# ivanacollg/MPC_CollisionAvoidance

Measured on AMD Instinct MI355X. Metric: batched SQP-RTI solves/sec (USV, N=40 horizon, 10 obstacles), higher is better.
Workload: dtype f64

## Files before the change

### include/usvmpc.h

```cpp
#ifndef USVMPC_H
#define USVMPC_H

#include <stddef.h>

#ifdef __cplusplus
extern "C" {
#endif

#define USVMPC_NX_MAX 14
#define USVMPC_NU_MAX 2
#define USVMPC_NY_MAX 16
#define USVMPC_K_MAX 32

enum { USVMPC_MODEL_USV = 0,
       USVMPC_MODEL_GUIDANCE_CA1 = 1,
       USVMPC_MODEL_PF_CA = 2,
       USVMPC_MODEL_GENERATED = 3 };

enum { USVMPC_HPIPM_BALANCE = 0, USVMPC_HPIPM_SPEED = 1, USVMPC_HPIPM_ROBUST = 2, USVMPC_HPIPM_R04 = 3 };

enum { USVMPC_E_ARG = -1, USVMPC_E_FIELD = -2, USVMPC_E_STAGE = -3, USVMPC_E_SIZE = -4,
       USVMPC_E_HIP = -5, USVMPC_E_NODEVICE = -6 };

typedef struct usvmpc_desc {
// ... 13 lines not shown
    double uh[USVMPC_K_MAX];
    int soft;
    double lsh[USVMPC_K_MAX], ush[USVMPC_K_MAX];
    double zl[USVMPC_K_MAX], zu[USVMPC_K_MAX], Zl[USVMPC_K_MAX], Zu[USVMPC_K_MAX];
    int qp_iter_max;
    double mu0, thr0, tol_stat, tol_eq, tol_ineq, tol_comp, alpha_min;
    int sbx[USVMPC_NX_MAX];
    double lsbx[USVMPC_NX_MAX], usbx[USVMPC_NX_MAX];
    double zl_bx[USVMPC_NX_MAX], zu_bx[USVMPC_NX_MAX], Zl_bx[USVMPC_NX_MAX], Zu_bx[USVMPC_NX_MAX];
    int sim_num_steps;
    int nlp_max_iter;
    double nlp_tol_stat, nlp_tol_eq, nlp_tol_ineq, nlp_tol_comp;
    int hpipm_mode;
    int cond_pred_corr;
    double cpc_factor;
} usvmpc_desc;

typedef struct usvmpc_handle usvmpc_handle;

int usvmpc_model_dims(int model, int *nx, int *nu);
void usvmpc_default_options(usvmpc_desc *d);
int usvmpc_hpipm_profile(usvmpc_desc *d, int mode);

int usvmpc_create(const usvmpc_desc *d, usvmpc_handle **out);
int usvmpc_destroy(usvmpc_handle *h);

int usvmpc_set(usvmpc_handle *h, const char *field, int stage, const double *v, size_t n);
int usvmpc_get(usvmpc_handle *h, const char *field, int stage, double *out, size_t n);
int usvmpc_obstacles_step(usvmpc_handle *h, double T);
int usvmpc_get_int(usvmpc_handle *h, const char *field, int *out);
// ... 3 lines not shown
int usvmpc_solve_async(usvmpc_handle *h);
int usvmpc_sync(usvmpc_handle *h);

int usvmpc_get_device_ptr(usvmpc_handle *h, const char *field, void **dptr);
int usvmpc_last_kernel_ms(usvmpc_handle *h, float *linearize_ms, float *qp_ms);
int usvmpc_kernel_ms(usvmpc_handle *h, int n, float *linearize_ms, float *qp_ms);
int usvmpc_tick_ms(usvmpc_handle *h, int n, float *ms);
int usvmpc_fail_counts(usvmpc_handle *h, int n, int *counts);
int usvmpc_unconverged_counts(usvmpc_handle *h, int n, int *counts);
int usvmpc_unconverged_total(usvmpc_handle *h, long long *total);
int usvmpc_handover_counts(usvmpc_handle *h, int n, int *counts);
int usvmpc_followup_ms(usvmpc_handle *h, int n, float *ms);
int usvmpc_handover_co_counts(usvmpc_handle *h, int n, int *finished, int *timeouts);
int usvmpc_pipeline_stats(usvmpc_handle *h, long *used, long *discarded);
int usvmpc_lin_pair_launches(usvmpc_handle *h, long *launches);
int usvmpc_last_mapping(usvmpc_handle *h, int *mapping);
int usvmpc_advance(usvmpc_handle *h, double sigma, unsigned long long seed);
int usvmpc_set_stream(usvmpc_handle *h, void *stream);
int usvmpc_set_option(usvmpc_handle *h, const char *name, double value);
int usvmpc_guidance_reset(usvmpc_handle *h, const double *waypoints, int npts, const double *psi);
int usvmpc_guidance_prepare(usvmpc_handle *h, const double *vel_uv, const double *pose, const double *obstacles,
                            const int *n_obstacles, int lmax);
int usvmpc_guidance_sense(usvmpc_handle *h, const double *pose, const double *world, int n_world, double max_radius,
                          double *obstacles, int *n_obstacles);
int usvmpc_guidance_publish(usvmpc_handle *h, double *heading, double *r_des, double *speed, double *ye, int *active);
int usvmpc_guidance_state(usvmpc_handle *h, int *wp_index, float *past_psied);
int usvmpc_pf_reset(usvmpc_handle *h, const double *waypoints, int npts);
int usvmpc_pf_world(usvmpc_handle *h, const double *world, int n_world, double max_radius);
int usvmpc_pf_prepare(usvmpc_handle *h, const double *vel_uvr, const double *pose);
int usvmpc_pf_publish(usvmpc_handle *h, double *thr_port, double *thr_stbd, double *Tx, double *Tz, float *e_u, float *e_ye, double *speed,
// ... 34 lines not shown
```

### mpc_collisionavoidance_amd/_capi.py

```python
import ctypes as C
import os
import sys

import numpy as np

NXM, NUM, NYM, KM = 14, 2, 16, 32
MODEL_IDS = {"usv_model": 0, "usv_model_guidance_ca1": 1, "usv_model_pf_ca": 2}
MODEL_DIMS = {0: (5, 2), 1: (8, 1), 2: (14, 2)}

_dp = C.POINTER(C.c_double)
_ip = C.POINTER(C.c_int)


class Desc(C.Structure):
    _fields_ = [("model", C.c_int), ("N", C.c_int), ("Tf", C.c_double), ("K", C.c_int),
                ("batch", C.c_int), ("device", C.c_int),
                ("W", C.c_double * (NYM * NYM)), ("W_e", C.c_double * (NXM * NXM)),
                ("Vx", C.c_double * (NYM * NXM)), ("Vu", C.c_double * (NYM * NUM)),
                ("Vx_e", C.c_double * (NXM * NXM)),
                ("nbu", C.c_int), ("idxbu", C.c_int * NUM), ("lbu", C.c_double * NUM), ("ubu", C.c_double * NUM),
                ("nbx", C.c_int), ("idxbx", C.c_int * NXM), ("lbx", C.c_double * NXM), ("ubx", C.c_double * NXM),
                ("uh", C.c_double * KM), ("soft", C.c_int),
                ("lsh", C.c_double * KM), ("ush", C.c_double * KM),
                ("zl", C.c_double * KM), ("zu", C.c_double * KM), ("Zl", C.c_double * KM), ("Zu", C.c_double * KM),
                ("qp_iter_max", C.c_int), ("mu0", C.c_double), ("thr0", C.c_double),
                ("tol_stat", C.c_double), ("tol_eq", C.c_double), ("tol_ineq", C.c_double),
                ("tol_comp", C.c_double), ("alpha_min", C.c_double),
                ("sbx", C.c_int * NXM), ("lsbx", C.c_double * NXM), ("usbx", C.c_double * NXM),
                ("zl_bx", C.c_double * NXM), ("zu_bx", C.c_double * NXM), ("Zl_bx", C.c_double * NXM), ("Zu_bx", C.c_double * NXM),
                ("sim_num_steps", C.c_int), ("nlp_max_iter", C.c_int),
                ("nlp_tol_stat", C.c_double), ("nlp_tol_eq", C.c_double), ("nlp_tol_ineq", C.c_double),
                ("nlp_tol_comp", C.c_double),
                ("hpipm_mode", C.c_int), ("cond_pred_corr", C.c_int), ("cpc_factor", C.c_double)]


class SimDesc(C.Structure):
    _fields_ = [("model", C.c_int), ("batch", C.c_int), ("device", C.c_int), ("T", C.c_double), ("num_steps", C.c_int),
                ("sens_forw", C.c_int)]


HPIPM_MODES = {"BALANCE": 0, "SPEED": 1, "ROBUST": 2, "R04": 3}


def lib_path():
    return os.environ.get("USVMPC_LIB") or os.path.join(os.path.dirname(os.path.abspath(__file__)), "csrc", "libusvmpc.so")


loaded_before_torch = False

EXPORTS = ["usvmpc_model_dims", "usvmpc_default_options", "usvmpc_hpipm_profile", "usvmpc_create", "usvmpc_destroy",
           "usvmpc_set", "usvmpc_get", "usvmpc_get_int", "usvmpc_solve", "usvmpc_solve_sqp", "usvmpc_solve_async",
           "usvmpc_sync", "usvmpc_get_device_ptr", "usvmpc_last_kernel_ms", "usvmpc_kernel_ms", "usvmpc_tick_ms", "usvmpc_fail_counts", "usvmpc_unconverged_counts", "usvmpc_unconverged_total", "usvmpc_handover_counts", "usvmpc_handover_co_counts", "usvmpc_followup_ms", "usvmpc_pipeline_stats", "usvmpc_lin_pair_launches", "usvmpc_last_mapping",
           "usvmpc_advance", "usvmpc_set_stream", "usvmpc_set_option", "usvmpc_calibrate_traffic", "usvmpc_guidance_reset", "usvmpc_guidance_prepare", "usvmpc_guidance_sense",
           "usvmpc_guidance_publish", "usvmpc_guidance_state", "usvmpc_device_bytes", "usvmpc_last_error",
           "usvmpc_debug_model_eval", "usvmpc_debug_obstacle_eval",
           "usvmpc_sim_create", "usvmpc_sim_destroy", "usvmpc_sim_set", "usvmpc_sim_solve", "usvmpc_sim_get", "usvmpc_sim_get_device_ptr",
           "usvmpc_sim_set_stream", "usvmpc_sim_last_error", "usvmpc_advance_sim", "usvmpc_obstacles_step",
           "usvmpc_pf_reset", "usvmpc_pf_world", "usvmpc_pf_prepare", "usvmpc_pf_publish", "usvmpc_pf_state",
           "usvmpc_pf_world_vel", "usvmpc_pf_world_step", "usvmpc_pf_world_read"]


_libs = {}


def load(path):
    global loaded_before_torch
    path = os.path.abspath(path)
# ... 21 lines not shown
    L.usvmpc_solve_sqp.argtypes = [C.c_void_p, _ip]
    L.usvmpc_solve_async.argtypes = [C.c_void_p]
    L.usvmpc_sync.argtypes = [C.c_void_p]
    L.usvmpc_get_device_ptr.argtypes = [C.c_void_p, C.c_char_p, C.POINTER(C.c_void_p)]
    L.usvmpc_last_kernel_ms.argtypes = [C.c_void_p, C.POINTER(C.c_float), C.POINTER(C.c_float)]
    L.usvmpc_kernel_ms.argtypes = [C.c_void_p, C.c_int, C.POINTER(C.c_float), C.POINTER(C.c_float)]
    L.usvmpc_tick_ms.argtypes = [C.c_void_p, C.c_int, C.POINTER(C.c_float)]
    L.usvmpc_fail_counts.argtypes = [C.c_void_p, C.c_int, _ip]
    L.usvmpc_unconverged_counts.argtypes = [C.c_void_p, C.c_int, _ip]
    L.usvmpc_handover_counts.argtypes = [C.c_void_p, C.c_int, _ip]
    L.usvmpc_unconverged_total.argtypes = [C.c_void_p, C.POINTER(C.c_longlong)]
    L.usvmpc_handover_co_counts.argtypes = [C.c_void_p, C.c_int, _ip, _ip]
    L.usvmpc_followup_ms.argtypes = [C.c_void_p, C.c_int, C.POINTER(C.c_float)]
    L.usvmpc_pipeline_stats.argtypes = [C.c_void_p, C.POINTER(C.c_long), C.POINTER(C.c_long)]
    L.usvmpc_lin_pair_launches.argtypes = [C.c_void_p, C.POINTER(C.c_long)]
    L.usvmpc_last_mapping.argtypes = [C.c_void_p, C.POINTER(C.c_int)]
    L.usvmpc_advance.argtypes = [C.c_void_p, C.c_double, C.c_ulonglong]
    L.usvmpc_set_stream.argtypes = [C.c_void_p, C.c_void_p]
    L.usvmpc_set_option.argtypes = [C.c_void_p, C.c_char_p, C.c_double]
    L.usvmpc_calibrate_traffic.argtypes = [C.c_void_p, C.c_int, _dp, _dp]
    L.usvmpc_guidance_reset.argtypes = [C.c_void_p, _dp, C.c_int, _dp]
    L.usvmpc_guidance_prepare.argtypes = [C.c_void_p, _dp, _dp, _dp, _ip, C.c_int]
    L.usvmpc_guidance_sense.argtypes = [C.c_void_p, _dp, _dp, C.c_int, C.c_double, _dp, _ip]
    L.usvmpc_guidance_publish.argtypes = [C.c_void_p, _dp, _dp, _dp, _dp, _ip]
    L.usvmpc_guidance_state.argtypes = [C.c_void_p, _ip, C.POINTER(C.c_float)]
    _fp = C.POINTER(C.c_float)
    L.usvmpc_pf_reset.argtypes = [C.c_void_p, _dp, C.c_int]
    L.usvmpc_pf_world.argtypes = [C.c_void_p, _dp, C.c_int, C.c_double]
    L.usvmpc_pf_prepare.argtypes = [C.c_void_p, _dp, _dp]
    L.usvmpc_pf_publish.argtypes = [C.c_void_p, _dp, _dp, _dp, _dp, _fp, _fp, _dp, _ip]
# ... 193 lines not shown
```

### mpc_collisionavoidance_amd/acados_template.py

```python
import ctypes as C

import numpy as np

from . import _capi


class SymVec:

    def __init__(self, n, names=None):
        self.n = int(n)
        self.names = list(names) if names is not None else ["v%d" % i for i in range(self.n)]

    def size(self):
        return (self.n, 1)

    @property
    def shape(self):
        return (self.n, 1)

    def __len__(self):
        return self.n

    def __sub__(self, other):
        return self
# ... 280 lines not shown
            return np.zeros(0)
        a = (C.c_float * (n - 1))()
        self._check(self._lib.usvmpc_tick_ms(self._h, n, a))
        return np.array(a[:])

    def fail_counts(self, n):
        a = (C.c_int * n)()
        self._check(self._lib.usvmpc_fail_counts(self._h, n, a))
        return np.array(a[:])

    def pipeline_stats(self):
        a, b = C.c_long(), C.c_long()
        self._check(self._lib.usvmpc_pipeline_stats(self._h, C.byref(a), C.byref(b)))
        return a.value, b.value

    def lin_pair_launches(self):
        a = C.c_long()
        self._check(self._lib.usvmpc_lin_pair_launches(self._h, C.byref(a)))
        return a.value

    def last_mapping(self):
        a = C.c_int()
        self._check(self._lib.usvmpc_last_mapping(self._h, C.byref(a)))
        return a.value

    def unconverged_counts(self, n):
        a = (C.c_int * n)()
        self._check(self._lib.usvmpc_unconverged_counts(self._h, n, a))
        return np.array(a[:])

# ... 357 lines not shown
```

### mpc_collisionavoidance_amd/csrc/gfx950/lanes.hpp

```cpp
#pragma once
#include <hip/hip_runtime.h>

#define USV_DEV __device__ __forceinline__

namespace lanes {

constexpr int GROUP = 16;

USV_DEV int lane() { return (int)(threadIdx.x & 15u); }
USV_DEV long group_linear() { return (long)blockIdx.x * (long)(blockDim.x >> 4) + (long)(threadIdx.x >> 4); }

template <int CTRL>
USV_DEV double dpp_mov(double v)
{
    const long l = __builtin_bit_cast(long, v);
    const long r = __builtin_amdgcn_update_dpp(0L, l, CTRL, 0xf, 0xf, true);
    return __builtin_bit_cast(double, r);
}

template <int K>
USV_DEV double bcast(double v)
{
    static_assert(K >= 0 && K < 16, "lane index");
    return dpp_mov<0x150 + K>(v);
// ... 191 lines not shown
    USV_DEV Planes(const double *base, unsigned nbytes, unsigned voff_) : voff(voff_)
    {
        rsrc = __builtin_amdgcn_make_buffer_rsrc(const_cast<double *>(base), 0, (int)nbytes, 0x00020000);
    }
    USV_DEV double ld(int plane) const
    {
        typedef unsigned u2 __attribute__((ext_vector_type(2)));
        const u2 v = __builtin_amdgcn_raw_buffer_load_b64(rsrc, (int)(voff + (unsigned)(plane * 128)), 0, PLANE_LOAD_AUX);
        return __builtin_bit_cast(double, v);
    }
    USV_DEV void st(int plane, double x) const
    {
        typedef unsigned u2 __attribute__((ext_vector_type(2)));
        __builtin_amdgcn_raw_buffer_store_b64(__builtin_bit_cast(u2, x), rsrc, (int)(voff + (unsigned)(plane * 128)), 0, PLANE_STORE_AUX);
    }
};

template <int NENT, int ROWS = 4, bool PERWAVE = false>
struct Xpose {
    USV_DEV static double *area()
    {
        __shared__ double s[NENT * ROWS];
        return s;
    }
    USV_DEV static unsigned row() { return PERWAVE ? (ROWS == 1 ? 0u : (threadIdx.x >> 6)) : ((threadIdx.x >> 4) & 3u); }
    USV_DEV static void put(int slot, double v) { area()[slot * ROWS + row()] = v; }
    USV_DEV static double get(int slot) { return area()[slot * ROWS + row()]; }
    USV_DEV static void sync() { __builtin_amdgcn_fence(__ATOMIC_RELEASE, "workgroup"); __builtin_amdgcn_wave_barrier(); __builtin_amdgcn_fence(__ATOMIC_ACQUIRE, "workgroup"); }
};

// ... 48 lines not shown
```

### mpc_collisionavoidance_amd/csrc/host_spec.hpp

```cpp
#pragma once
#include "../../include/usvmpc.h"
#include "params.hpp"
#include <cstring>
#include <cmath>
#include <string>

namespace usv {

inline int model_dims(int model, int &nx, int &nu)
{
    switch (model) {
    case USVMPC_MODEL_USV: nx = 5; nu = 2; return 0;
    case USVMPC_MODEL_GUIDANCE_CA1: nx = 8; nu = 1; return 0;
    case USVMPC_MODEL_PF_CA: nx = 14; nu = 2; return 0;
#ifdef USV_GEN_NX
    case USVMPC_MODEL_GENERATED: nx = USV_GEN_NX; nu = USV_GEN_NU; return 0;
#endif
    }
    return -1;
}

inline std::string build_spec(const usvmpc_desc &d, DevSpec &S)
{
    int nx, nu;
    if (model_dims(d.model, nx, nu)) return "unknown model id";
    if (d.N < 2) return "N must be >= 2";
    if (!(d.Tf > 0.0)) return "Tf must be positive";
    if (d.batch < 1) return "batch must be >= 1";
    if (d.K < 0 || d.K > KMAX) return "K out of range (0..32)";
    if (d.model == USVMPC_MODEL_USV && d.K != 0) return "model usv_model has no obstacle rows (K must be 0)";
    if (d.nbu < 0 || d.nbu > nu || d.nbx < 0 || d.nbx > nx) return "nbu/nbx out of range";
    {
        const double BIG = 1e100;
        for (int i = 0; i < d.nbu; i++) if (!(std::fabs(d.lbu[i]) <= BIG && std::fabs(d.ubu[i]) <= BIG)) return "lbu / ubu beyond 1e100 (or NaN)";
// ... 83 lines not shown
            S.box_dense = ndense > 0;
            S.aux_dense4 = 4 * ndense;
            int slot = k_last, j = 0;
            for (int r = 0; r < LANES; r++) {
                if (!S.has_b[r]) continue;
                if (slot < LANES) {
                    S.box_slot[r] = slot; S.box_step[r] = 0; S.slot_var[slot] = r; S.slot_is[slot] = 1; slot++;
                } else {
                    S.box_slot[r] = 4 * j; S.box_step[r] = 1;
                    for (int e = 0; e < 4; e++) { S.slot_var[4 * j + e] = r; S.slot_is[4 * j + e] = 2; }
                    j++;
                }
            }
        }
    }
    S.hdiag = 1;
    for (int i = 0; i < LANES; i++)
        for (int j = 0; j < LANES; j++)
            if (i != j && (S.Hc[i * LANES + j] != 0.0 || S.He[i * LANES + j] != 0.0)) S.hdiag = 0;
    S.nc = d.N * d.nbu * 2 + (d.N - 1) * (d.nbx * 2 + d.K * (d.soft ? 4 : 2));
    for (int i = 0; i < d.nbx; i++) S.nc += d.sbx[i] ? (d.N - 1) * 2 : 0;
    S.iter_max = d.qp_iter_max;
    S.mu0 = d.mu0; S.thr0 = d.thr0;
    S.tol_stat = d.tol_stat; S.tol_eq = d.tol_eq; S.tol_ineq = d.tol_ineq; S.tol_comp = d.tol_comp;
    S.alpha_min = d.alpha_min;
    if (S.iter_max < 1) return "qp_iter_max must be >= 1";
    if (d.sim_num_steps < 0 || d.sim_num_steps > 64) return "sim_num_steps out of range (1..64)";
    S.sim_steps = d.sim_num_steps > 0 ? d.sim_num_steps : 1;
    if (d.hpipm_mode < USVMPC_HPIPM_BALANCE || d.hpipm_mode > USVMPC_HPIPM_R04) return "hpipm_mode must be one of USVMPC_HPIPM_*";
    if (d.cpc_factor < 0.0) return "cpc_factor must be positive (0: the default, 2)";
// ... 43 lines not shown
```

### mpc_collisionavoidance_amd/csrc/params.hpp

```cpp
#pragma once
#include <type_traits>

namespace usv {

constexpr int LANES = 16;
constexpr int KMAX = 32;

struct DevSpec {
    double Hc[LANES * LANES];
    double He[LANES * LANES];
    double Mc[LANES * LANES];
    double Me[LANES * LANES];
    double lb[LANES], ub[LANES];
    int has_b[LANES];
    int boxpack;
    int boxpack_ok;
    int box_dense;
    int aux_dense4;
    int box_slot[LANES];
    int box_step[LANES];
    int slot_var[LANES];
    int slot_is[LANES];
    double uh[KMAX];
    double lsl[KMAX], lsu[KMAX];
// ... 5 lines not shown
    int p_static;
    int hdiag;
    int iter_max;
    double mu0, thr0, tol_stat, tol_eq, tol_ineq, tol_comp, alpha_min;
    int sim_steps;
    int npt;
    int any_bsoft;
    int bsoft[LANES];
    double b_zl[LANES], b_zu[LANES], b_Zl[LANES], b_Zu[LANES], b_lsl[LANES], b_lsu[LANES];
    double nlp_tol[4];
    int nbu, nbx, nsbx;
    int box_pos[LANES];
    int sbx_pos[LANES];
    int cpc;
    double cpc_factor;
};

template <class M>
struct MatPack {
    static constexpr int NX = M::NX, NU = M::NU, NZ = NX + NU;
    static constexpr unsigned row_mask(int j) { return M::SENS[j]; }
    static constexpr int count(int j) { return __builtin_popcount(M::SENS[j]); }
    static constexpr int start(int j)
    {
        int s = 0;
        for (int i = 0; i < j; i++) s += __builtin_popcount(M::SENS[i]);
        return s;
    }
    static constexpr bool diag_one(int j) { return ((M::DIAG_ONE >> j) & 1u) != 0u; }
    static constexpr unsigned col_mask()
    {
        unsigned m = 0;
        for (int j = 0; j < NX; j++) m |= M::SENS[j];
        return m;
    }
    static constexpr int NE = start(NX);
    static constexpr int NPK = (NE + 15) / 16;
    static constexpr int nth(unsigned mask, int i)
    {
        for (int b = 0; b < 32; b++)
            if ((mask >> b) & 1u) {
                if (i == 0) return b;
                i--;
            }
        return 0;
    }
    static constexpr int rank(unsigned mask, int b) { return __builtin_popcount(mask & ((1u << b) - 1u)); }
    static constexpr bool consistent()
    {
        unsigned cols = 0;
        for (int j = 0; j < NX; j++) {
            cols |= M::SENS[j];
// ... 135 lines not shown
```

### mpc_collisionavoidance_amd/csrc/qp_ipm.hpp

```cpp
#pragma once
#include "lanes.hpp"
#include "params.hpp"
#include "sfor.hpp"

#pragma clang fp contract(on)

namespace usv {

template <bool SOFTROW, bool MIXED = false>
struct RowCalc {
    double ll, lu, tl, tu, sl, su, lsl, lsu, tsl, tsu;
    double dl, du, zl, zu, Zl, Zu, bsl, bsu;
    bool act, soft;
    double rdl, rdu, rsl, rsu, rdsl, rdsu;
    USV_DEV bool is_soft() const
    {
        if constexpr (!SOFTROW) return false;
        else if constexpr (MIXED) return soft;
        else return true;
    }
    double itl, itu, itsl, itsu;
    double Gl, Gu, iDl, iDu, rhol, rhou;
    double ml, mu, msl, msu;
    double dll, dlu, dtl, dtu, dsl, dsu, dlsl, dlsu, dtsl, dtsu;
// ... 212 lines not shown
    bool auxlive;
    long stage_stride;
    unsigned stage_bytes;
    bool xlane, ulane, valid, isPX, isPY;
    bool ounit;
    static constexpr unsigned CMASK = MP::col_mask();
    static constexpr int NCOL = __builtin_popcount(CMASK);
    static constexpr int ZSLOT = MP::NPK * 16, OSLOT = ZSLOT + 1;
    using XP = lanes::Xpose<MP::NPK * 16 + 2, (WIDE ? WW : 4), WIDE>;
    unsigned rowtab[(NX + 3) / 4], coltab[(NCOL + 3) / 4];
    bool selfone;
    bool isslot, isdense, anydense;
    bool slot_u;
    int bsrc, bstep, ssrc;
    bool hasb;
    static constexpr int KC = KCH > 0 ? KCH : 1;
    enum : int {
        ST_LB = 0, ST_UB, ST_HDS, ST_HDT, ST_UH, ST_OX = ST_UH + KC, ST_OY = ST_OX + KC, ST_LH = ST_OY + KC, ST_SOFT = ST_LH + KC,
        ST_ZL = ST_SOFT, ST_ZU = ST_ZL + (SOFT ? KC : 0), ST_QL = ST_ZU + (SOFT ? KC : 0), ST_QU = ST_QL + (SOFT ? KC : 0),
        ST_BSL = ST_QU + (SOFT ? KC : 0), ST_BSU = ST_BSL + (SOFT ? KC : 0), ST_BOX = ST_BSU + (SOFT ? KC : 0),
        ST_SLOT = ST_BOX + (SOFTBOX ? 6 : 0),
        ST_CPC = ST_SLOT + (MERGE ? 2 : 0),
        ST_N = ST_CPC + (CPC ? 1 : 0)
    };
    using ST = lanes::Stash<ST_N, (WIDE ? 16 : 64)>;
    struct CRef {
        int slot;
        USV_DEV operator double() const { return ST::get(slot); }
        USV_DEV void operator=(double v) const { ST::put(slot, v); }
    };
// ... 63 lines not shown
            bool so = false;
            sfor<0, NX>([&](auto j) {
                if constexpr (MP::diag_one(j) && ((CMASK >> (NU + j)) & 1u) == 0u) so = (lane == NU + j) ? true : so;
            });
            selfone = so;
            XP::put(ZSLOT, 0.0);
            XP::put(OSLOT, 1.0);
        }
        isslot = PACK && S.slot_is[lane] == 1;
        isdense = PACK && S.slot_is[lane] == 2;
        anydense = PACK && lanes::uniform(S.box_dense) != 0;
        bsrc = S.box_slot[lane];
        bstep = S.box_step[lane];
        ssrc = S.slot_var[lane];
        slot_u = isslot && ssrc < NU;
        if constexpr (MERGE) {
            slot_lb = S.lb[isslot ? ssrc : 0];
            slot_ub = S.ub[isslot ? ssrc : 0];
        }
        lbv = S.lb[lane];
        ubv = S.ub[lane];
        hd_stage = S.Hc[lane * LANES + lane];
        hd_term = S.He[lane * LANES + lane];
        bsoft = SOFTBOX && S.bsoft[lane] != 0;
        if constexpr (SOFTBOX) {
            bzl = S.b_zl[lane]; bzu = S.b_zu[lane]; bZl = bsoft ? S.b_Zl[lane] : 1.0; bZu = bsoft ? S.b_Zu[lane] : 1.0;
            bbsl = S.b_lsl[lane]; bbsu = S.b_lsu[lane];
        }
        if constexpr (KCH > 0) {
            sfor<0, KCH>([&](auto c) {
// ... 156 lines not shown
    {
        double a = isdense ? dense : 0.0;
        sfor<0, NU>([&](auto l) {
            const double r_l = lanes::bcast<l>(rg), u_l = lanes::bcast<l>(luv);
            a = (lane == AXL_RG - l) ? r_l : a;
            a = (lane == AXL_LU - l) ? u_l : a;
        });
        if constexpr (KCH > 0) a = (lane == AXL_ZX) ? zbx : ((lane == AXL_ZY) ? zby : a);
        return a;
    }
    USV_DEV double pos_sel(double zbx, double zby) const { return isPX ? zbx : (isPY ? zby : 0.0); }
    USV_DEV void mat_issue(int k, double *pk) const
    {
        const Planes W = ws(k);
        sfor<0, MP::NPK>([&](auto q) { pk[q] = W.ld(P_MAT + q); });
    }
    USV_DEV void mat_put(const double *pk) const
    {
        sfor<0, MP::NPK>([&](auto q) { XP::put(16 * q + lane, pk[q]); });
        XP::sync();
    }
    USV_DEV void mat_unpack(const double *pk, double *bat) const
    {
        mat_put(pk);
        sfor<0, NX>([&](auto j) {
            if constexpr (out_unit(j)) bat[j] = 0.0;
            else bat[j] = XP::get((int)((rowtab[j / 4] >> (8 * (j % 4))) & 0xffu));
        });
    }
    USV_DEV double mat_apply(const double *pk, double dz, double acc) const
// ... 104 lines not shown
        double bxs[SOFTBOX ? 6 : 1];
        double obs[KCH > 0 ? KCH : 1][OBSN];
        double raw[KCH > 0 ? KCH : 1][3];
    };
    enum : int { SW_BACK_A = 0, SW_FWD_A = 1, SW_BACK_B = 2, SW_FWD_B = 3 };

    template <int SW>
    USV_DEV void load_in(int k, StageIn &in) const
    {
        const Planes W = ws(k);
        in.z = W.ld(P_Z);
        in.aux = aux_ld(k, W);
        if constexpr (SW != SW_BACK_B) in.rb = (k < N) ? W.ld(P_RB0) : 0.0;
        if constexpr (SW == SW_BACK_A) {
            in.dz = W.ld(P_DZ);
            in.dza = W.ld(P_DZA);
            in.gq = W.ld(P_GQ);
        }
        if constexpr (SW == SW_BACK_B || SW == SW_FWD_B) in.dza = W.ld(P_DZA);
        if constexpr (SW == SW_BACK_B) in.pb = (k < N) ? W.ld(P_PB) : 0.0;
        if constexpr (SW != SW_BACK_A) {
            if (k < N) sfor<0, NU>([&](auto l) { in.lzu[l] = W.ld(P_LZU + l); });
            else sfor<0, NU>([&](auto l) { in.lzu[l] = 1.0; });
        }
        if constexpr (!PACK) {
            in.box[0] = W.ld(P_BLL); in.box[1] = W.ld(P_BLU); in.box[2] = W.ld(P_BTL); in.box[3] = W.ld(P_BTU);
            if constexpr (SOFTBOX) sfor<0, 6>([&](auto e) { in.bxs[e] = W.ld(P_BS + e); });
        }
        if constexpr (KCH > 0) {
            if (k >= 1 && k < N) {
                sfor<0, KCH>([&](auto c) {
                    sfor<0, OBSN>([&](auto e) { in.obs[c][e] = W.ld(P_OBS + c * OBSN + e); });
                    if (!pstat) obs_raw<c>(k, in.raw[c]);
                });
// ... 91 lines not shown
                }
                if (FACT && dfr_k < N) {
                    Wp.st(P_PB, dfr_pb);
                    sfor<0, NU>([&](auto l) { Wp.st(P_LZU + l, dfr_lz[l]); });
                }
            }
        };
        StageIn nxt;
        load_in<SW>(N, nxt);
        for (int k = N; k >= 0; k--) {
            const StageIn in = nxt;
            lanes::sched_fence();
            flush();
            const Planes W = ws(k);
            double mpk[MP::NPK];
            if (k < N) mat_issue(k, mpk);
            double z = in.z;
            const double zbx = aux_zx(in.aux), zby = aux_zy(in.aux);
            const double psel = pos_sel(zbx, zby);
            const double ou1 = ounit ? 1.0 : 0.0;
            const double *Hrow = (k < N ? S.Hc : S.He) + lane * LANES;
            const double hd = (k < N) ? hd_stage : hd_term;
            const double dza = FACT ? 0.0 : in.dza;
            double rb = FACT ? in.rb * rbscale : 0.0;
            BoxRow br;
            double Ghb = 0.0, gamb = 0.0, dlb = 0.0;
            const double dzp = FACT ? in.dz : 0.0, dzap = FACT ? in.dza : 0.0;
            double pk[4], dv = in.aux;
            const double znew = (FACT && pend) ? z + a_prev * dzp : z;
            if constexpr (!MERGE) {
                box_from(in, k, br);
                if (FACT) {
                    if (pend && br.act) {
                        chain<CPC>(br, z, true, dzap, sigmu_prev, Ghb, gamb, so_p);
                        br.expand(dzp);
                        br.apply(a_prev);
                        if constexpr (!PACK) box_store(W, br);
                    }
                }
                if constexpr (FACT && PACK) dv = box_pack(br, pk);
                chain<CPC>(br, znew, !FACT, dza, sigmu, Ghb, gamb, so_c);
                dlb = br.act ? br.ll - br.lu : 0.0;
// ... 199 lines not shown
        constexpr bool SUMS = !FINAL || CPC;
        double so_c = 1.0;
        if constexpr (CPC) so_c = so_cur;
        constexpr int SW = FINAL ? SW_FWD_B : SW_FWD_A;
        double dzx;
        {
            const Planes W0 = ws(0);
            dzx = xlane ? W0.ld(P_DX0) - W0.ld(P_Z) : 0.0;
        }
        double q = 1.0, s1 = 0.0, s2 = 0.0, dfr_dz = 0.0;
        StageIn nxt;
        load_in<SW>(0, nxt);
        for (int k = 0; k <= N; k++) {
            const StageIn in = nxt;
            lanes::sched_fence();
            if (k > 0) ws(k - 1).st(FINAL ? P_DZ : P_DZA, dfr_dz);
            const Planes W = ws(k);
            double mpk[MP::NPK];
            if (k < N) {
                mat_issue(k, mpk);
                load_in<SW>(k + 1, nxt);
            }
            double dz;
            const double zbx = aux_zx(in.aux), zby = aux_zy(in.aux);
            if (k < N) {
                double t[NU], du[NU];
                sfor<0, NU>([&](auto l) {
                    t[l] = lanes::bcast<AXL_LU - l>(in.aux) + lanes::gsum(xlane ? in.lzu[l] * dzx : 0.0);
                });
                sfor<0, NU>([&](auto qq) {
                    constexpr int l = NU - 1 - qq;
                    double acc = t[l];
                    sfor<l + 1, NU>([&](auto m) { acc -= lanes::bcast<m>(in.lzu[l]) * du[m]; });
                    du[l] = acc * lanes::bcast<l>(in.lzu[l]);
                });
                dz = xlane ? dzx : 0.0;
                sfor<0, NU>([&](auto l) { dz = (lane == l) ? -du[l] : dz; });
            } else {
                dz = xlane ? dzx : 0.0;
            }
            {
                const double z = in.z;
                const double dza = FINAL ? in.dza : dz;
                if constexpr (!MERGE) {
                    BoxRow br;
                    box_from(in, k, br);
                    double Gh, gam;
                    chain<CPC>(br, z, FINAL, dza, sigmu, Gh, gam, so_c);
                    br.expand(dz);
                    q = br.blocking(q);
                    if (SUMS && br.act) {
                        s1 += br.ll * br.dtl + br.tl * br.dll + br.lu * br.dtu + br.tu * br.dlu;
                        s2 += br.dll * br.dtl + br.dlu * br.dtu;
                        if constexpr (SOFTBOX) {
                            if (br.soft) {
                                s1 += br.lsl * br.dtsl + br.tsl * br.dlsl + br.lsu * br.dtsu + br.tsu * br.dlsu;
                                s2 += br.dlsl * br.dtsl + br.dlsu * br.dtsu;
                            }
// ... 12 lines not shown
                        o.expand(w);
                        q = o.blocking(q);
                        if (SUMS && o.act) {
                            s1 += o.ll * o.dtl + o.tl * o.dll + o.lu * o.dtu + o.tu * o.dlu;
                            s2 += o.dll * o.dtl + o.dlu * o.dtu;
                            if constexpr (SOFT) {
                                s1 += o.lsl * o.dtsl + o.tsl * o.dlsl + o.lsu * o.dtsu + o.tsu * o.dlsu;
                                s2 += o.dlsl * o.dtsl + o.dlsu * o.dtsu;
                            }
                        }
                    });
                }
            }
            dfr_dz = dz;
            if (k < N) {
                const double dxn = mat_apply(mpk, dz, in.rb * rbscale);
                dzx = xlane ? dxn : 0.0;
            }
        }
        ws(N).st(FINAL ? P_DZ : P_DZA, dfr_dz);
        alpha = 1.0 / lanes::gmax(q);
        if (SUMS) { S1 = lanes::gsum(s1); S2 = lanes::gsum(s2); }
    }

    enum : int { EX_GHB = 0, EX_GAMB, EX_DLB, EX_SC, EX_MU1, EX_MU2 = EX_MU1 + KC, EX_MU3 = EX_MU2 + KC, EX_MU4 = EX_MU3 + (SOFTBOX ? 1 : 0), EX_Z, EX_DV, EX_ALL };
    static constexpr int EX_FWD = 4 * KC + 2 + (SOFTBOX ? 2 : 0);
    static constexpr int EX_N = LDSWS ? ((int)EX_Z > EX_FWD ? (int)EX_Z : EX_FWD) : ((int)EX_ALL > EX_FWD ? (int)EX_ALL : EX_FWD);
    static_assert(!WIDE || EX_N == (LDSWS ? wide_ex_planes(KCH, SOFTBOX) : wide_ex_planes_hbm(KCH, SOFTBOX)), "host-side size of the exchange area");
    static constexpr int BS = 4 * WW;
    static constexpr int wide_lds_doubles(int N_) { return (LDSWS ? (N_ + 1) * NPLW * LANES : 0) + BS * EX_N * LANES + (WW > 1 ? LANES : 0); }
    USV_DEV static void wide_sync()
    {
        if constexpr (WW > 1) lanes::block_sync();
        else lanes::lds_fence();
    }
// ... 780 lines not shown
            }
            wide_sync();
        }
    }
    static constexpr bool HAS_CPC = CPC;
    static constexpr bool CAN_SUSPEND = !WIDE && !LDSWS && HDIAG && !SOFTBOX && ((PACK && KCH == 1) || (!PACK && KCH == 0));
    USV_DEV void suspend(bool sel, int it, double a_prev, double sig_prev)
    {
        if constexpr (AUXLDS) {
            for (int k = 0; k <= N; k++) {
                const Planes W = ws(k);
                const double a = aux_ld(k, W);
                if (sel) W.st(P_AUX, a);
            }
        }
        if (sel && lane == 0) {
            double *r = P.susp_rec + 4 * b;
            double itv = (double)it;
            if constexpr (CPC) itv = ((double)so_prv == 0.0) ? -itv : itv;
            r[0] = a_prev; r[1] = sig_prev; r[2] = rbscale; r[3] = itv;
        }
        const bool co = P.co_ctl != nullptr;
        if (co) lanes::release_agent();
        if (sel && lane == 0) {
            const int slot = lanes::fetch_add(P.susp_count);
            if (co) lanes::publish(P.susp_list + slot, (int)g);
            else P.susp_list[slot] = (int)g;
        }
    }

// ... 157 lines not shown
```

### mpc_collisionavoidance_amd/csrc/usvmpc.hip

```cpp
#ifndef USV_PART
#define USV_PART -1
#endif
#define USV_MAIN (USV_PART <= 0)

#include "gfx950/lanes.hpp"

#include "guidance.hpp"
#include "host_spec.hpp"
#include "linearize.hpp"
#include "models.hpp"
#include "obstacle_tracks.hpp"
#include "pf_guidance.hpp"
#include "qp_ipm.hpp"
#include "sim.hpp"
#include "cond_launch.hpp"
#ifdef USV_GEN_MODEL_HEADER
#include USV_GEN_MODEL_HEADER
#endif

#include <algorithm>
#include <cstdint>
#include <cstdio>
#include <cstring>
#include <mutex>
// ... 634 lines not shown
    bool extern_access;
    bool pipeline;
    hipStream_t aux_stream;
    hipEvent_t ev_pre, ev_spec;
    int *d_epoch, *d_redo, *d_perm2, *d_inv;
    long spec_for;
    bool spec_valid;
    bool spec_outstanding;
    int spec_quiet;
    long spec_hits, spec_misses;
    const int *spec_perm;
    bool spec_fine;
    int lin_force;
    int lin_pairs;
    long lin_pair_launches;
    int *d_force_epoch, *d_force_redo, *d_force_inv;
    int cond_N2;
    CondDims cond_dims;
    CondDims *d_cond_dims;
    double *d_cond_scratch;
    long cond_teams;
    size_t cond_lds;
    double *d_obs_pos, *d_obs_vel;
    double *d_clear, *d_clear_min;
    bool tracks_on;
    bool tracks_pos_set;
    bool tracks_dirty;
    bool tracks_extern;
    bool step_on_advance;
    bool clear_reset;
// ... 645 lines not shown
        hand = h->resume_cap > 0 && hand_it > 0;
    }
    h->ptrs.susp_count = hand ? h->d_susp_count + h->nsolves % usvmpc_handle::RING : nullptr;
    h->ptrs.susp_list = hand ? h->d_susp_list : nullptr;
    h->ptrs.susp_rec = hand ? h->d_susp_rec : nullptr;
    h->ptrs.handover_iter = hand ? hand_it : 0;
    const dim3 qg((unsigned)((ng * LANES + qp_block - 1) / qp_block)), qb(qp_block);
    const bool co = hand && h->handover_co != 0 && h->resume_lds && k.resume_co != nullptr && h->own_stream && co_prepare(h);
    if (co) {
        HIP_TRY(h, set_dynamic_lds((const void *)k.resume_co, xbytes));
        h->ptrs.co_ctl = h->d_co_ctl + 8 * (h->nsolves % usvmpc_handle::RING);
        HIP_TRY(h, hipMemsetAsync(h->ptrs.co_ctl, 0, 8 * sizeof(int), h->stream));
        HIP_TRY(h, hipMemsetAsync(h->d_susp_list, 0xff, (size_t)h->B * sizeof(int), h->stream));
        HIP_TRY(h, hipEventRecord(h->ev_co_pre, h->stream));
    }
    hipLaunchKernelGGL(kern, qg, qb, aux_bytes, h->stream, h->ptrs, ng, phase, q0, 4);
    if (co) {
        hipLaunchKernelGGL(usv_co_done, dim3(1), dim3(1), 0, h->stream, h->ptrs.co_ctl);
        HIP_TRY(h, hipStreamWaitEvent(h->co_stream, h->ev_co_pre, 0));
        long nco = std::min<long>(h->resume_cap, (long)h->B);
        nco = std::min<long>(nco, h->co_wgs > 0 ? (long)h->co_wgs : (long)std::max(h->ncu, 1));
        hipLaunchKernelGGL(k.resume_co, dim3((unsigned)nco), dim3(qp_block), xbytes, h->co_stream, h->ptrs, (int)qg.x, (int)h->B, h->co_spin_limit);
        HIP_TRY(h, hipEventRecord(h->ev_co_end, h->co_stream));
    }
    if (hand) {
        HIP_TRY(h, hipEventRecord(ev[3], h->stream));
        h->ev3_set[h->nsolves % usvmpc_handle::RING] = true;
        const long nwg = std::min<long>(h->resume_cap, (long)h->B);
        hipLaunchKernelGGL(kern_resume, dim3((unsigned)nwg), dim3(qp_block), xbytes, h->stream, h->ptrs);
    }
// ... 293 lines not shown
void sim_launch_model(usvmpc_sim *s)
{
    const long B = s->B;
    if (s->sens) {
        const long threads = B * LANES;
        hipLaunchKernelGGL((usv_sim<M, true>), dim3((unsigned)((threads + 255) / 256)), dim3(256), 0, s->stream, s->x, s->u, s->xn, s->S, B, s->T,
                           s->num_steps);
    } else {
        hipLaunchKernelGGL((usv_sim<M, false>), dim3((unsigned)((B + 255) / 256)), dim3(256), 0, s->stream, s->x, s->u, s->xn, s->S, B, s->T,
                           s->num_steps);
    }
}

}

extern "C" {

int usvmpc_model_dims(int model, int *nx, int *nu)
{
    int a, b;
    if (model_dims(model, a, b)) return USVMPC_E_ARG;
    if (nx) *nx = a;
    if (nu) *nu = b;
    return 0;
}

void usvmpc_default_options(usvmpc_desc *d)
{
    if (d) default_options(*d);
}
// ... 47 lines not shown
    h->soft = d->soft != 0 || d->model == USVMPC_MODEL_GUIDANCE_CA1;
#ifdef USV_GEN_MODEL_HEADER
    if (d->model == USVMPC_MODEL_GENERATED) { h->kch = USV_GEN_KCH; h->soft = USV_GEN_SOFT != 0; }
#endif
    h->device = d->device;
    h->bytes = 0; h->nsolves = 0; h->own_stream = true;
    h->map_changed = false;
    h->export_at = -1;
    h->layout_dirty = false;
    h->last_cond = false;
    h->pipeline = true;
    h->aux_stream = nullptr; h->ev_pre = nullptr; h->ev_spec = nullptr;
    h->d_epoch = nullptr; h->d_redo = nullptr; h->d_perm2 = nullptr; h->d_inv = nullptr;
    h->spec_fine = false;
    h->lin_pairs = model_has_pairs(h->desc.model) ? 1 : 0; h->lin_pair_launches = 0;
    h->lin_force = 0; h->d_force_epoch = nullptr; h->d_force_redo = nullptr; h->d_force_inv = nullptr;
    h->spec_for = -1; h->spec_valid = false; h->spec_outstanding = false; h->spec_perm = nullptr;
    h->spec_quiet = 0; h->spec_hits = 0; h->spec_misses = 0;
    h->noise_mask = ~0u;
    h->instance_offset = 0;
    h->d_obs_pos = nullptr; h->d_obs_vel = nullptr; h->d_clear = nullptr; h->d_clear_min = nullptr;
    h->tracks_on = false; h->tracks_pos_set = false; h->tracks_dirty = false; h->tracks_extern = false;
    h->step_on_advance = true; h->clear_reset = false;
    h->cond_N2 = 0; h->d_cond_dims = nullptr; h->d_cond_scratch = nullptr; h->cond_teams = 0; h->cond_lds = 0;
    h->dynamic_rows = true;
    h->qp_cap = 0;
    h->aux_lds = true;
    h->aux_cap = 0;
    h->lds_mode = -1;
    h->lds_cap = 0;
// ... 424 lines not shown
int usvmpc_pipeline_stats(usvmpc_handle *h, long *used, long *discarded)
{
    if (!h) return USVMPC_E_ARG;
    if (used) *used = h->spec_hits;
    if (discarded) *discarded = h->spec_misses;
    return 0;
}

int usvmpc_lin_pair_launches(usvmpc_handle *h, long *launches)
{
    if (!h || !launches) return USVMPC_E_ARG;
    *launches = h->lin_pair_launches;
    return 0;
}

int usvmpc_last_mapping(usvmpc_handle *h, int *mapping)
{
    if (!h || !mapping) return USVMPC_E_ARG;
    *mapping = h->last_wide;
    return 0;
}

int usvmpc_last_kernel_ms(usvmpc_handle *h, float *linearize_ms, float *qp_ms)
{
    return usvmpc_kernel_ms(h, 1, linearize_ms, qp_ms);
}

static int pf_apply_static(usvmpc_handle *h);

int usvmpc_advance(usvmpc_handle *h, double sigma, unsigned long long seed)
// ... 202 lines not shown
        reset_caps(h);
        return 0;
    }
    if (s == "host_mirror") {
        if (value != 0.0) { if (!h->mirror) { h->err = "host_mirror cannot be switched on again"; return USVMPC_E_ARG; } return 0; }
        if (!h->mirror) return 0;
        HIP_TRY(h, hipSetDevice(h->device));
        const int rcf = mirror_flush(h);
        if (rcf) return rcf;
        HIP_TRY(h, hipStreamSynchronize(h->stream));
        h->inflight = false; h->out_valid = false;
        (void)hipHostFree(h->mirror);
        h->mirror = nullptr;
        return 0;
    }
    if (s == "static_obstacles" || s == "pack_box_rows") {
        if (s == "static_obstacles") { h->spec.p_static = value != 0.0; h->tracks_dirty = true; }
        else { h->spec.boxpack = (value != 0.0 && h->spec.boxpack_ok) ? 1 : 0; reset_caps(h); h->layout_dirty = true; }
        HIP_TRY(h, hipSetDevice(h->device));
        HIP_TRY(h, hipMemcpyAsync(h->d_spec, &h->spec, sizeof(DevSpec), hipMemcpyHostToDevice, h->stream));
        HIP_TRY(h, hipStreamSynchronize(h->stream));
        return 0;
    }
    h->err = "unknown option '" + s + "'";
    return USVMPC_E_FIELD;
}

static int guidance_alloc(usvmpc_handle *h, int npts)
{
    if (h->desc.model != USVMPC_MODEL_GUIDANCE_CA1) { h->err = "the guidance front end belongs to usv_model_guidance_ca1"; return USVMPC_E_ARG; }
    HIP_TRY(h, hipSetDevice(h->device));
    const size_t B = h->B;
// ... 572 lines not shown
```

Baseline: 1.022 million.

## Pack dza plane into idle lanes of last matrix plane in QP sweeps

Stores the predictor step direction (dza) in the unused padding lanes of the last packed dynamics-matrix plane, so one plane load during the backward and forward sweeps serves both the matrix and dza. The value is scattered and gathered across lanes with lane-permute tables built on the host, and a write-through store keeps it out of cache. This removes one plane load and one store per stage per sweep, at the cost of extra cross-lane gathers, a model-dependent lane layout and a reconstruction pass that writes P_DZA back on exit. It is on by default when the layout fits and can be disabled by a desc field or option.

```diff
diff --git a/include/usvmpc.h b/include/usvmpc.h
--- a/include/usvmpc.h
+++ b/include/usvmpc.h
@@ -51,6 +51,7 @@
     int hpipm_mode;
     int cond_pred_corr;
     double cpc_factor;
+    int dza_ride_off;
 } usvmpc_desc;
 
 typedef struct usvmpc_handle usvmpc_handle;
@@ -84,6 +85,7 @@
 int usvmpc_handover_co_counts(usvmpc_handle *h, int n, int *finished, int *timeouts);
 int usvmpc_pipeline_stats(usvmpc_handle *h, long *used, long *discarded);
 int usvmpc_lin_pair_launches(usvmpc_handle *h, long *launches);
+int usvmpc_dza_ride_launches(usvmpc_handle *h, long *launches);
 int usvmpc_last_mapping(usvmpc_handle *h, int *mapping);
 int usvmpc_advance(usvmpc_handle *h, double sigma, unsigned long long seed);
 int usvmpc_set_stream(usvmpc_handle *h, void *stream);
diff --git a/mpc_collisionavoidance_amd/_capi.py b/mpc_collisionavoidance_amd/_capi.py
--- a/mpc_collisionavoidance_amd/_capi.py
+++ b/mpc_collisionavoidance_amd/_capi.py
@@ -31,7 +31,8 @@
                 ("sim_num_steps", C.c_int), ("nlp_max_iter", C.c_int),
                 ("nlp_tol_stat", C.c_double), ("nlp_tol_eq", C.c_double), ("nlp_tol_ineq", C.c_double),
                 ("nlp_tol_comp", C.c_double),
-                ("hpipm_mode", C.c_int), ("cond_pred_corr", C.c_int), ("cpc_factor", C.c_double)]
+                ("hpipm_mode", C.c_int), ("cond_pred_corr", C.c_int), ("cpc_factor", C.c_double),
+                ("dza_ride_off", C.c_int)]
 
 
 class SimDesc(C.Structure):
@@ -50,7 +51,7 @@
 
 EXPORTS = ["usvmpc_model_dims", "usvmpc_default_options", "usvmpc_hpipm_profile", "usvmpc_create", "usvmpc_destroy",
            "usvmpc_set", "usvmpc_get", "usvmpc_get_int", "usvmpc_solve", "usvmpc_solve_sqp", "usvmpc_solve_async",
-           "usvmpc_sync", "usvmpc_get_device_ptr", "usvmpc_last_kernel_ms", "usvmpc_kernel_ms", "usvmpc_tick_ms", "usvmpc_fail_counts", "usvmpc_unconverged_counts", "usvmpc_unconverged_total", "usvmpc_handover_counts", "usvmpc_handover_co_counts", "usvmpc_followup_ms", "usvmpc_pipeline_stats", "usvmpc_lin_pair_launches", "usvmpc_last_mapping",
+           "usvmpc_sync", "usvmpc_get_device_ptr", "usvmpc_last_kernel_ms", "usvmpc_kernel_ms", "usvmpc_tick_ms", "usvmpc_fail_counts", "usvmpc_unconverged_counts", "usvmpc_unconverged_total", "usvmpc_handover_counts", "usvmpc_handover_co_counts", "usvmpc_followup_ms", "usvmpc_pipeline_stats", "usvmpc_lin_pair_launches", "usvmpc_dza_ride_launches", "usvmpc_last_mapping",
            "usvmpc_advance", "usvmpc_set_stream", "usvmpc_set_option", "usvmpc_calibrate_traffic", "usvmpc_guidance_reset", "usvmpc_guidance_prepare", "usvmpc_guidance_sense",
            "usvmpc_guidance_publish", "usvmpc_guidance_state", "usvmpc_device_bytes", "usvmpc_last_error",
            "usvmpc_debug_model_eval", "usvmpc_debug_obstacle_eval",
@@ -102,6 +103,8 @@
     L.usvmpc_followup_ms.argtypes = [C.c_void_p, C.c_int, C.POINTER(C.c_float)]
     L.usvmpc_pipeline_stats.argtypes = [C.c_void_p, C.POINTER(C.c_long), C.POINTER(C.c_long)]
     L.usvmpc_lin_pair_launches.argtypes = [C.c_void_p, C.POINTER(C.c_long)]
+    if hasattr(L, "usvmpc_dza_ride_launches"):
+        L.usvmpc_dza_ride_launches.argtypes = [C.c_void_p, C.POINTER(C.c_long)]
     L.usvmpc_last_mapping.argtypes = [C.c_void_p, C.POINTER(C.c_int)]
     L.usvmpc_advance.argtypes = [C.c_void_p, C.c_double, C.c_ulonglong]
     L.usvmpc_set_stream.argtypes = [C.c_void_p, C.c_void_p]
diff --git a/mpc_collisionavoidance_amd/acados_template.py b/mpc_collisionavoidance_amd/acados_template.py
--- a/mpc_collisionavoidance_amd/acados_template.py
+++ b/mpc_collisionavoidance_amd/acados_template.py
@@ -318,6 +318,11 @@
         self._check(self._lib.usvmpc_pipeline_stats(self._h, C.byref(a), C.byref(b)))
         return a.value, b.value
 
+    def dza_ride_launches(self):
+        a = C.c_long(0)
+        self._check(self._lib.usvmpc_dza_ride_launches(self._h, C.byref(a)))
+        return int(a.value)
+
     def lin_pair_launches(self):
         a = C.c_long()
         self._check(self._lib.usvmpc_lin_pair_launches(self._h, C.byref(a)))
diff --git a/mpc_collisionavoidance_amd/csrc/gfx950/lanes.hpp b/mpc_collisionavoidance_amd/csrc/gfx950/lanes.hpp
--- a/mpc_collisionavoidance_amd/csrc/gfx950/lanes.hpp
+++ b/mpc_collisionavoidance_amd/csrc/gfx950/lanes.hpp
@@ -229,6 +229,12 @@
         typedef unsigned u2 __attribute__((ext_vector_type(2)));
         __builtin_amdgcn_raw_buffer_store_b64(__builtin_bit_cast(u2, x), rsrc, (int)(voff + (unsigned)(plane * 128)), 0, PLANE_STORE_AUX);
     }
+#define USV_LANES_ST_THROUGH 1
+    USV_DEV void st_through(int plane, double x) const
+    {
+        typedef unsigned u2 __attribute__((ext_vector_type(2)));
+        __builtin_amdgcn_raw_buffer_store_b64(__builtin_bit_cast(u2, x), rsrc, (int)(voff + (unsigned)(plane * 128)), 0, 16);
+    }
 };
 
 template <int NENT, int ROWS = 4, bool PERWAVE = false>
diff --git a/mpc_collisionavoidance_amd/csrc/host_spec.hpp b/mpc_collisionavoidance_amd/csrc/host_spec.hpp
--- a/mpc_collisionavoidance_amd/csrc/host_spec.hpp
+++ b/mpc_collisionavoidance_amd/csrc/host_spec.hpp
@@ -18,6 +18,29 @@
 #endif
     }
     return -1;
+}
+
+constexpr void model_ride(int model, int &cap, int &first, int &ipx, int &ipy)
+{
+    cap = 0; first = 0; ipx = 0; ipy = 0;
+    switch (model) {
+    case USVMPC_MODEL_USV: cap = 9; first = 7; break;
+    case USVMPC_MODEL_GUIDANCE_CA1: cap = 4; first = 12; ipx = 5; ipy = 6; break;
+    case USVMPC_MODEL_PF_CA: cap = 9; first = 7; ipx = 10; ipy = 11; break;
+    }
+}
+
+inline void ride_layout(DevSpec &S, int cap, int first, unsigned need, bool off)
+{
+    S.ride_cap = cap; S.ride_first = first;
+    S.ride_need = __builtin_popcount(need & 0xffffu);
+    for (int r = 0; r < LANES; r++) { S.ride_var[r] = -1; S.ride_at[r] = -1; }
+    S.dza_ride_ok = (cap > 0 && first + cap == LANES && S.ride_need <= cap) ? 1 : 0;
+    S.dza_ride = (S.dza_ride_ok && !off) ? 1 : 0;
+    if (!S.dza_ride_ok) return;
+    int l = first;
+    for (int r = 0; r < LANES; r++)
+        if ((need >> r) & 1u) { S.ride_var[l] = r; S.ride_at[r] = l; l++; }
 }
 
 inline std::string build_spec(const usvmpc_desc &d, DevSpec &S)
@@ -131,6 +154,14 @@
             }
         }
     }
+    {
+        int cap, first, ipx, ipy;
+        model_ride(d.model, cap, first, ipx, ipy);
+        unsigned need = 0;
+        for (int r = 0; r < LANES; r++)
+            if (S.has_b[r] != 0 || (d.K > 0 && (r == nu + ipx || r == nu + ipy))) need |= 1u << r;
+        ride_layout(S, cap, first, need, d.dza_ride_off != 0);
+    }
     S.hdiag = 1;
     for (int i = 0; i < LANES; i++)
         for (int j = 0; j < LANES; j++)
diff --git a/mpc_collisionavoidance_amd/csrc/params.hpp b/mpc_collisionavoidance_amd/csrc/params.hpp
--- a/mpc_collisionavoidance_amd/csrc/params.hpp
+++ b/mpc_collisionavoidance_amd/csrc/params.hpp
@@ -43,6 +43,12 @@
     int sbx_pos[LANES];
     int cpc;
     double cpc_factor;
+    int dza_ride;
+    int dza_ride_ok;
+    int ride_cap, ride_need;
+    int ride_first;
+    int ride_var[LANES];
+    int ride_at[LANES];
 };
 
 template <class M>
@@ -65,6 +71,8 @@
     }
     static constexpr int NE = start(NX);
     static constexpr int NPK = (NE + 15) / 16;
+    static constexpr int IDLE = NPK * 16 - NE;
+    static constexpr int IDLE0 = NE % 16;
     static constexpr int nth(unsigned mask, int i)
     {
         for (int b = 0; b < 32; b++)
diff --git a/mpc_collisionavoidance_amd/csrc/qp_ipm.hpp b/mpc_collisionavoidance_amd/csrc/qp_ipm.hpp
--- a/mpc_collisionavoidance_amd/csrc/qp_ipm.hpp
+++ b/mpc_collisionavoidance_amd/csrc/qp_ipm.hpp
@@ -250,6 +250,10 @@
     bool slot_u;
     int bsrc, bstep, ssrc;
     bool hasb;
+    static constexpr bool RIDE_OK = !WIDE && !LDSWS && MP::IDLE > 0;
+    enum : int { P_MATL = WL::P_MAT + MP::NPK - 1 };
+    bool ride;
+    int ridetab;
     static constexpr int KC = KCH > 0 ? KCH : 1;
     enum : int {
         ST_LB = 0, ST_UB, ST_HDS, ST_HDT, ST_UH, ST_OX = ST_UH + KC, ST_OY = ST_OX + KC, ST_LH = ST_OY + KC, ST_SOFT = ST_LH + KC,
@@ -343,6 +347,13 @@
         bstep = S.box_step[lane];
         ssrc = S.slot_var[lane];
         slot_u = isslot && ssrc < NU;
+        ride = false;
+        ridetab = 0;
+        if constexpr (RIDE_OK) {
+            ride = lanes::uniform(S.dza_ride) != 0 && lanes::uniform(S.ride_first) == MP::IDLE0;
+            const int at = S.ride_at[lane], var = S.ride_var[lane];
+            ridetab = (at >= 0 ? at : 0) | ((var >= 0 ? var : 0) << 4) | (lane >= MP::IDLE0 ? 256 : 0);
+        }
         if constexpr (MERGE) {
             slot_lb = S.lb[isslot ? ssrc : 0];
             slot_ub = S.ub[isslot ? ssrc : 0];
@@ -529,6 +540,41 @@
     {
         const Planes W = ws(k);
         sfor<0, MP::NPK>([&](auto q) { pk[q] = W.ld(P_MAT + q); });
+    }
+    USV_DEV void mat_issue(int k, double *pk, double pre) const
+    {
+        if constexpr (RIDE_OK) {
+            const Planes W = ws(k);
+            sfor<0, MP::NPK - 1>([&](auto q) { pk[q] = W.ld(P_MAT + q); });
+            if (ride) pk[MP::NPK - 1] = pre;
+            else pk[MP::NPK - 1] = W.ld(P_MATL);
+        } else {
+            mat_issue(k, pk);
+        }
+    }
+    USV_DEV double dza_ld(int k, const Planes &W) const
+    {
+        if constexpr (RIDE_OK) {
+            if (ride) return (k < N) ? W.ld(P_MATL) : 0.0;
+        }
+        return W.ld(P_DZA);
+    }
+    USV_DEV void ride_st(int k, double v) const
+    {
+        if constexpr (RIDE_OK) {
+#ifdef USV_LANES_ST_THROUGH
+            ws(k).st_through(P_MATL, v);
+#else
+            ws(k).st(P_MATL, v);
+#endif
+        }
+    }
+    USV_DEV double dza_take(double v) const
+    {
+        if constexpr (RIDE_OK) {
+            if (ride) return lanes::gather(v, ridetab);
+        }
+        return v;
     }
     USV_DEV void mat_put(const double *pk) const
     {
@@ -663,10 +709,10 @@
         if constexpr (SW != SW_BACK_B) in.rb = (k < N) ? W.ld(P_RB0) : 0.0;
         if constexpr (SW == SW_BACK_A) {
             in.dz = W.ld(P_DZ);
-            in.dza = W.ld(P_DZA);
+            in.dza = dza_ld(k, W);
             in.gq = W.ld(P_GQ);
         }
-        if constexpr (SW == SW_BACK_B || SW == SW_FWD_B) in.dza = W.ld(P_DZA);
+        if constexpr (SW == SW_BACK_B || SW == SW_FWD_B) in.dza = dza_ld(k, W);
         if constexpr (SW == SW_BACK_B) in.pb = (k < N) ? W.ld(P_PB) : 0.0;
         if constexpr (SW != SW_BACK_A) {
             if (k < N) sfor<0, NU>([&](auto l) { in.lzu[l] = W.ld(P_LZU + l); });
@@ -788,18 +834,19 @@
             flush();
             const Planes W = ws(k);
             double mpk[MP::NPK];
-            if (k < N) mat_issue(k, mpk);
+            if (k < N) mat_issue(k, mpk, in.dza);
             double z = in.z;
             const double zbx = aux_zx(in.aux), zby = aux_zy(in.aux);
             const double psel = pos_sel(zbx, zby);
+            const double dzs = dza_take(in.dza);
             const double ou1 = ounit ? 1.0 : 0.0;
             const double *Hrow = (k < N ? S.Hc : S.He) + lane * LANES;
             const double hd = (k < N) ? hd_stage : hd_term;
-            const double dza = FACT ? 0.0 : in.dza;
+            const double dza = FACT ? 0.0 : dzs;
             double rb = FACT ? in.rb * rbscale : 0.0;
             BoxRow br;
             double Ghb = 0.0, gamb = 0.0, dlb = 0.0;
-            const double dzp = FACT ? in.dz : 0.0, dzap = FACT ? in.dza : 0.0;
+            const double dzp = FACT ? in.dz : 0.0, dzap = FACT ? dzs : 0.0;
             double pk[4], dv = in.aux;
             const double znew = (FACT && pend) ? z + a_prev * dzp : z;
             if constexpr (!MERGE) {
@@ -1029,11 +1076,16 @@
         for (int k = 0; k <= N; k++) {
             const StageIn in = nxt;
             lanes::sched_fence();
-            if (k > 0) ws(k - 1).st(FINAL ? P_DZ : P_DZA, dfr_dz);
+            if (k > 0) {
+                if (FINAL) ws(k - 1).st(P_DZ, dfr_dz);
+                else if (ride) ride_st(k - 1, dfr_dz);
+                else ws(k - 1).st(P_DZA, dfr_dz);
+            }
             const Planes W = ws(k);
             double mpk[MP::NPK];
             if (k < N) {
-                mat_issue(k, mpk);
+                if constexpr (FINAL) mat_issue(k, mpk, in.dza);
+                else mat_issue(k, mpk);
                 load_in<SW>(k + 1, nxt);
             }
             double dz;
@@ -1056,7 +1108,8 @@
             }
             {
                 const double z = in.z;
-                const double dza = FINAL ? in.dza : dz;
+                double dza = dz;
+                if constexpr (FINAL) dza = dza_take(in.dza);
                 if constexpr (!MERGE) {
                     BoxRow br;
                     box_from(in, k, br);
@@ -1099,11 +1152,18 @@
             }
             dfr_dz = dz;
             if (k < N) {
+                if constexpr (RIDE_OK && !FINAL) {
+                    if (ride) {
+                        const double gz = lanes::gather(dz, ridetab >> 4);
+                        dfr_dz = (ridetab & 256) ? gz : mpk[MP::NPK - 1];
+                    }
+                }
                 const double dxn = mat_apply(mpk, dz, in.rb * rbscale);
                 dzx = xlane ? dxn : 0.0;
             }
         }
-        ws(N).st(FINAL ? P_DZ : P_DZA, dfr_dz);
+        if (FINAL) ws(N).st(P_DZ, dfr_dz);
+        else if (!ride) ws(N).st(P_DZA, dfr_dz);
         alpha = 1.0 / lanes::gmax(q);
         if (SUMS) { S1 = lanes::gsum(s1); S2 = lanes::gsum(s2); }
     }
@@ -1914,6 +1974,15 @@
                 if (sel) W.st(P_AUX, a);
             }
         }
+        if constexpr (RIDE_OK) {
+            if (ride) {
+                for (int k = 0; k <= N; k++) {
+                    const Planes W = ws(k);
+                    const double a = (k < N) ? dza_take(W.ld(P_MATL)) : 0.0;
+                    if (sel) W.st(P_DZA, a);
+                }
+            }
+        }
         if (sel && lane == 0) {
             double *r = P.susp_rec + 4 * b;
             double itv = (double)it;
diff --git a/mpc_collisionavoidance_amd/csrc/usvmpc.hip b/mpc_collisionavoidance_amd/csrc/usvmpc.hip
--- a/mpc_collisionavoidance_amd/csrc/usvmpc.hip
+++ b/mpc_collisionavoidance_amd/csrc/usvmpc.hip
@@ -672,6 +672,7 @@
     int lin_force;
     int lin_pairs;
     long lin_pair_launches;
+    long dza_ride_launches;
     int *d_force_epoch, *d_force_redo, *d_force_inv;
     int cond_N2;
     CondDims cond_dims;
@@ -1347,6 +1348,7 @@
         HIP_TRY(h, hipMemsetAsync(h->d_susp_list, 0xff, (size_t)h->B * sizeof(int), h->stream));
         HIP_TRY(h, hipEventRecord(h->ev_co_pre, h->stream));
     }
+    if (h->spec.dza_ride) h->dza_ride_launches++;
     hipLaunchKernelGGL(kern, qg, qb, aux_bytes, h->stream, h->ptrs, ng, phase, q0, 4);
     if (co) {
         hipLaunchKernelGGL(usv_co_done, dim3(1), dim3(1), 0, h->stream, h->ptrs.co_ctl);
@@ -1670,6 +1672,18 @@
 
 }
 
+#ifndef USV_GEN_ONLY
+template <class M>
+constexpr bool ride_table_ok(int model)
+{
+    int cap = 0, first = 0, ipx = 0, ipy = 0;
+    model_ride(model, cap, first, ipx, ipy);
+    return cap == MatPack<M>::IDLE && first == MatPack<M>::IDLE0 && ipx == M::IPX && ipy == M::IPY;
+}
+static_assert(ride_table_ok<ModelM0>(USVMPC_MODEL_USV) && ride_table_ok<ModelM1>(USVMPC_MODEL_GUIDANCE_CA1) && ride_table_ok<ModelM2>(USVMPC_MODEL_PF_CA),
+              "model_ride (host_spec.hpp) disagrees with MatPack / the models' position states");
+#endif
+
 extern "C" {
 
 int usvmpc_model_dims(int model, int *nx, int *nu)
@@ -1747,6 +1761,7 @@
     h->d_epoch = nullptr; h->d_redo = nullptr; h->d_perm2 = nullptr; h->d_inv = nullptr;
     h->spec_fine = false;
     h->lin_pairs = model_has_pairs(h->desc.model) ? 1 : 0; h->lin_pair_launches = 0;
+    h->dza_ride_launches = 0;
     h->lin_force = 0; h->d_force_epoch = nullptr; h->d_force_redo = nullptr; h->d_force_inv = nullptr;
     h->spec_for = -1; h->spec_valid = false; h->spec_outstanding = false; h->spec_perm = nullptr;
     h->spec_quiet = 0; h->spec_hits = 0; h->spec_misses = 0;
@@ -2201,6 +2216,13 @@
     return 0;
 }
 
+int usvmpc_dza_ride_launches(usvmpc_handle *h, long *launches)
+{
+    if (!h || !launches) return USVMPC_E_ARG;
+    *launches = h->dza_ride_launches;
+    return 0;
+}
+
 int usvmpc_last_mapping(usvmpc_handle *h, int *mapping)
 {
     if (!h || !mapping) return USVMPC_E_ARG;
@@ -2433,8 +2455,9 @@
         h->mirror = nullptr;
         return 0;
     }
-    if (s == "static_obstacles" || s == "pack_box_rows") {
+    if (s == "static_obstacles" || s == "pack_box_rows" || s == "dza_ride") {
         if (s == "static_obstacles") { h->spec.p_static = value != 0.0; h->tracks_dirty = true; }
+        else if (s == "dza_ride") { h->spec.dza_ride = (value != 0.0 && h->spec.dza_ride_ok) ? 1 : 0; h->layout_dirty = true; }
         else { h->spec.boxpack = (value != 0.0 && h->spec.boxpack_ok) ? 1 : 0; reset_caps(h); h->layout_dirty = true; }
         HIP_TRY(h, hipSetDevice(h->device));
         HIP_TRY(h, hipMemcpyAsync(h->d_spec, &h->spec, sizeof(DevSpec), hipMemcpyHostToDevice, h->stream));
```

New measurement: 998,100. 0.977x the previous value.
